# delehef/asgart

Hardware: AMD Instinct MI355X
Metric: Mbp/s probe+extend (direct+RC, k=20 g=100) (higher is better)
Workload: dtype u64 keys / u32 SA

## Files before the change

asgart_amd/csrc/call_front.hpp:

```cpp
#pragma once
#include "search_call.hpp"

namespace asgart {

__global__ void stall_kernel(unsigned long long ticks) {
    const unsigned long long t0 = wall_clock64();
    while (wall_clock64() - t0 < ticks) __builtin_amdgcn_s_sleep(100);
}

struct ProbeBuffer {
    DevBuf Workspace::*buf;
    size_t (*bytes)(uint64_t W, bool wide);
};
static const ProbeBuffer kProbeBuffers[7] = {
    {&Workspace::p_lo, [](uint64_t W, bool wide) { return (size_t)W * (wide ? 8 : 4); }},
    {&Workspace::p_raw, [](uint64_t W, bool) { return (size_t)W * 4; }},
    {&Workspace::p_filt, [](uint64_t W, bool) { return (size_t)W * 4; }},
    {&Workspace::row_off, [](uint64_t W, bool) { return ((size_t)W + 1) * 8; }},
    {&Workspace::blk, [](uint64_t W, bool) { return (size_t)((W + kScanTile - 1) / kScanTile + 4) * sizeof(ScanEl); }},
    {&Workspace::big_list, [](uint64_t W, bool) { return (size_t)W * 4; }},
    {&Workspace::rank_list, [](uint64_t W, bool) { return (size_t)W * 4; }},
};

int32_t reserve_probe_workspace(asgart_index *idx, SearchCtx &cx, uint64_t W) {
    Workspace &w = cx.ws;
    for (const ProbeBuffer &pb : kProbeBuffers)
        if (pb.buf != &Workspace::rank_list || idx->d_sap) RC_TRY((w.*pb.buf).reserve(pb.bytes(W, idx->wide)));
    RC_TRY(w.counters.reserve(CT_COUNT * 8));
    return 0;
}

bool carve_probe_workspace(asgart_index *idx, const uint64_t *Wc) {
    if (idx->ws_arena.p) return false;
    size_t off = 0;
    struct Piece {
        DevBuf *b;
// ... 26 lines not shown
    const uint32_t n_blk = rp.n_tiles((uint32_t)kScanTile);
    const uint64_t seg_cap = (uint64_t)W_probes / (rp.tstar + 1) + (uint64_t)n_chunks + 64;
    RC_TRY(reserve_probe_workspace(idx, cx, W));
    RC_TRY(w.seg_list.reserve((size_t)seg_cap * 4));
    RC_TRY(w.counters.reserve(CT_COUNT * 8));
    d_ctr = w.counters.as<unsigned long long>();
    HIP_TRY(hipMemsetAsync(d_ctr, 0, CT_COUNT * 8, s));
    ix = idx->template view<SlotT>();
    p_lo = w.p_lo.as<SlotT>() - rp.g_lo;
    p_raw = w.p_raw.as<uint32_t>() - rp.g_lo;
    p_filt = w.p_filt.as<uint32_t>() - rp.g_lo;
    row_off = w.row_off.as<unsigned long long>() - rp.g_lo;
    unsigned long long *scan_desc = w.blk.as<unsigned long long>();
    uint32_t *big_list = w.big_list.as<uint32_t>();
    uint32_t *rank_list = w.rank_list.as<uint32_t>();
    seg_list = w.seg_list.as<uint32_t>();

    if (opt.test_stall_s > 0) stall_kernel<<<1, 64, 0, s>>>((unsigned long long)opt.test_stall_s * 100000000ull);
    HIP_TRY(hipEventRecord(cx.ev[EV_SEARCH], s));
    probe_count_kernel<SlotT, false><<<rp.n_tiles((uint32_t)kProbeBlock), kProbeThreads, 0, s>>>(
        ix, rp, p_lo, p_raw, p_filt, big_list, rank_list, d_ctr);
    HIP_TRY(hipEventRecord(cx.ev[EV_PROBE_COUNT], s));
    collect_pending_kernel<<<std::min<uint32_t>(rp.n_tiles((uint32_t)kCollectTile), 256u * 8u), kCollectBlock, 0, s>>>(
        rp, p_filt, big_list, rank_list, d_ctr);
    big_count_kernel<SlotT, false><<<2048, 256, 0, s>>>(ix, rp, p_lo, p_raw, p_filt, big_list, d_ctr);
    uint32_t *const ranked_top = big_list + W;
    if (ix.sap)
        rank_count_kernel<SlotT, false><<<2048, 256, 0, s>>>(ix, rp, p_lo, p_raw, p_filt, rank_list, big_list, ranked_top,
                                                             ix.sar ? idx->ranked_fill : 0, d_ctr);
    HIP_TRY(hipEventRecord(cx.ev[EV_SEARCHED], s));
    HIP_TRY(hipMemsetAsync(scan_desc, 0, (size_t)n_blk * 16, s));
    scan_segments_kernel<<<std::min<uint32_t>(n_blk, 256u * 2u), kScanBlock, 0, s>>>(rp, p_filt, scan_desc, n_blk, row_off, seg_list, d_ctr);
    HIP_TRY(hipEventRecord(cx.ev[EV_SCANNED], s));
    HIP_TRY(hipGetLastError());
    HIP_TRY(hipMemcpyAsync(h_ctr, d_ctr, kCtrBytes, hipMemcpyDeviceToHost, s));
    RC_TRY(wd_sync(idx, cx, s, "the probe search and the scans"));
    total_hits = h_ctr[CT_TOTAL_HITS];
    n_seg = h_ctr[CT_SEG];
    if (h_ctr[CT_AMBIG]) {
// ... 49 lines not shown
```

asgart_amd/csrc/call_place.hpp:

```cpp
#pragma once
#include "search_call.hpp"

namespace asgart {

template <class SlotT>
int32_t SearchCall<SlotT>::place() {
    rec_cap = std::max<uint64_t>(1u << 18, w.fam_sds.cap / sizeof(SdRec));
    RC_TRY(w.ovf_list.reserve((size_t)(n_seg + 1) * 4 * kTiers));
    h_recs = nullptr;
    n_hrec = 0;
    const int force_tier = (int)opt.force_tier;
    RC_TRY(w.seg_keys.reserve((size_t)n_seg * 4 * 2));
    RC_TRY(w.seg_vals.reserve((size_t)n_seg * 4 * 2));
    uint32_t *kbuf = w.seg_keys.as<uint32_t>(), *vbuf = w.seg_vals.as<uint32_t>();
    HIP_TRY(hipMemsetAsync(d_ctr + CT_N1, 0, (size_t)(CT_COUNT - CT_N1) * 8, s));
    arms_kernel = rp.C <= (uint64_t)kHitBatch && opt.arms_kernel != 0 && (uint64_t)idx->n < (1ull << 42);
    for (int t = 1; t <= kTiers; ++t) {
        const TierShape &sh = shape(t);
        const bool usable = sh.kernel != TierKernel::none && !(arms_kernel && rp.C > (uint64_t)sh.hits);
        tier_cap[t] = usable ? (uint32_t)((uint64_t)sh.cap() * (uint64_t)(sh.widen ? opt.*sh.widen : 100) / 100u) : 0u;
    }
    tier_cap[kTiers] = 0xFFFFFFFFu;
    if (arms_kernel)
        tier_cap[3] = std::min(std::max(shape(3).cap(), tier_cap[6]), tier_cap[3]);
// ... 46 lines not shown
    int force_eff = force_tier;
    while (force_eff > 1 && force_eff < kTiers && !tier_enabled(force_eff)) ++force_eff;
    pp.sum1 = kTier1MaxSum;
    pp.force_tier = force_eff;
    {
        uint32_t *long_list = w.ovf_list.as<uint32_t>();
        seg_stats_lanes_kernel<<<(unsigned)std::min<uint64_t>((n_seg + 63) / 64, 256ull * 9ull * 2ull), 64, 0, s>>>(
            rp, p_filt, seg_list, d_ctr + CT_SEG, kbuf, vbuf, pp, long_list, d_ctr);
        seg_stats_kernel<<<(unsigned)std::min<uint64_t>(n_seg, 256ull * 16ull), 64, 0, s>>>(
            rp, p_filt, seg_list, d_ctr + CT_LONGSEG, long_list, kbuf, vbuf, pp, d_ctr);
    }
    HIP_TRY(hipGetLastError());
    HIP_TRY(hipStreamWaitEvent(s, cx.ev[EV_HIT_ROWS], 0));
    if (cluster_barren) {
        HIP_TRY(hipEventRecord(cx.ev[EV_BARREN], s));
        cluster_barren_kernel<SlotT, 16384><<<256 * 32, 64, 0, s>>>(rp, pp, row_off, hits, seg_list, d_ctr + CT_SEG, kbuf, 1u, 1024u,
                                                                   d_ctr + CT_CLUSTER_CUR, d_ctr);
        HIP_TRY(hipEventRecord(cx.ev[EV_BARREN_SMALL], s));
        cluster_barren_kernel<SlotT, 131072><<<256 * 9, 64, 0, s>>>(rp, pp, row_off, hits, seg_list, d_ctr + CT_SEG, kbuf, 1025u,
                                                                   16384u, d_ctr + CT_CLUSTER_CUR + 1, d_ctr);
        HIP_TRY(hipGetLastError());
        HIP_TRY(hipEventRecord(cx.ev[EV_BARREN_BIG], s));
    }
    if (split_on) {
        SplitParams sp{};
        sp.range_len = (uint32_t)opt.split_len;
        sp.warm = (uint32_t)opt.split_warm;
        sp.min_span = (uint32_t)std::min<int64_t>(opt.split_min, 0x7FFFFFFF);
        sp.max_runs = kMaxRuns - kMaxSplits;
        sp.max_cuts = kMaxCuts;
        sp.max_splits = kMaxSplits;
        {
            BlockedSeg *h_blocked = reinterpret_cast<BlockedSeg *>(h_split + kOffBlocked);
            std::lock_guard<std::mutex> lk(idx->mu);
            sp.n_blocked = blocked_in_call(idx->split_blocked, call_sig, rp.modes, n_passes, lo_lim, hi_lim, kSplitBlockedMax,
                                           [&](int32_t p_, const SplitVerdict &b) {
                                               *h_blocked++ = BlockedSeg{(uint32_t)p_ * K + ((uint32_t)b.key - lo_lim), b.range_len, b.allowed, b.warm};
// ... 80 lines not shown
        fprintf(stderr, "[asgart] %u long segment(s) cut into ranges: %u runs (ranges of %llu probes%s), %u cuts to check\n",
                n_splits, n_runs, (unsigned long long)h_split_hdr[4], opt.split_len ? "" : ": the shortest that keeps the runs within the budget", n_cuts);
    if (opt.debug) {
        fprintf(stderr, "[asgart] %llu segments, %llu walked wave by wave; per tier:", (unsigned long long)n_seg,
                (unsigned long long)h_ctr[CT_LONGSEG]);
        unsigned long long placed = 0;
        for (int t = 0; t < kTiers; ++t) {
            fprintf(stderr, " %llu", (unsigned long long)n_t[t]);
            placed += n_t[t];
        }
        fprintf(stderr, "; %llu barren (no arm can reach min_duplication_length: not run), %llu of them by the positions of their hits\n",
                (unsigned long long)n_seg - placed, (unsigned long long)h_ctr[CT_CLUSTER_BARREN]);
        fprintf(stderr, "[asgart] tail rule: thresholds (hits) of tiers 2, 4, 5: %u %u %u; %llu segment(s) moved to the next tier that holds more\n",
                pp.tail_hits[1], pp.tail_hits[3], pp.tail_hits[4], (unsigned long long)h_ctr[CT_TAIL_UP]);
        if (cluster_barren) {
            float ms_a = 0.f, ms_b = 0.f, ms_p = 0.f;
            (void)hipEventElapsedTime(&ms_a, cx.ev[EV_BARREN], cx.ev[EV_BARREN_SMALL]);
            (void)hipEventElapsedTime(&ms_b, cx.ev[EV_BARREN_SMALL], cx.ev[EV_BARREN_BIG]);
            (void)hipEventElapsedTime(&ms_p, cx.ev[EV_FILL], cx.ev[EV_BARREN]);
            fprintf(stderr, "[asgart] hit rows filled, placement walk beside it: %.2f ms; barren by position: segments of up to 1 024 hits %.2f ms, up to 16 384 hits %.2f ms\n",
                    ms_p, ms_a, ms_b);
        }
    }
    for (int t = 0; t < kTiers; ++t) ovf[t] = w.ovf_list.as<uint32_t>() + (size_t)t * (n_seg + 1);
    heavy_cap64 = (std::max<uint64_t>((uint64_t)rp.C * ((uint64_t)rp.tstar + 1u) + 64u, 4096u) + 3u) & ~3ull;
    if (heavy_cap64 >= (1ull << 24)) {
        set_error("max_cardinality * (max_gap_size / step + 1) = %llu live arms per segment: more than 2^24 are not supported",
                  (unsigned long long)heavy_cap64);
        return ASGART_E_CAP;
    }
    const size_t per_wg7 = (size_t)heavy_cap64 * (4 * sizeof(SlotT) + 28);
    const size_t per_wg6 = (size_t)caph * (4 * sizeof(SlotT) + 16);
    const size_t per_wg = std::max(per_wg6, per_wg7);
    n_wg7 = (unsigned)std::max<uint64_t>(1, std::min<uint64_t>(256, (16ull << 30) / (4 * per_wg)));
    region = std::max(per_wg6 * 256, per_wg * (size_t)n_wg7);
    RC_TRY(w.scratch.reserve(region * 4));
// ... 7 lines not shown
```

asgart_amd/csrc/call_stats.hpp:

```cpp
#pragma once
#include "search_call.hpp"

using namespace asgart;

template <class F>
static void by_slot(const asgart_index *idx, F f) {
    if (idx->wide) f(uint64_t{});
    else f(uint32_t{});
}

extern "C" {

int32_t asgart_tier_segments(asgart_index *idx, uint64_t *out) {
    if (!idx || !out) {
        set_error("bad argument");
        return ASGART_E_ARG;
    }
    idx->acquire_all();
    const SearchCtx &cx = idx->ctx[idx->last_ctx];
    for (int i = 0; i < 8; ++i) out[i] = cx.has_last ? cx.tier_segments[i] : 0;
    idx->release_all();
    return 0;
}

// ... 115 lines not shown
            }
            const unsigned g = rp.n_tiles(256u);
            by_slot(idx, [&](auto slot_tag) {
                using SlotT = decltype(slot_tag);
                yardstick_kernel<SlotT><<<g, 256, 0, s>>>(idx->view<SlotT>(), rp, cx.ws.p_filt.as<uint32_t>() - rp.g_lo, d_ctr);
            });
            HIP_TRY(hipGetLastError());
            HIP_TRY(hipMemsetAsync(d_ctr + CT_ALG_BYTES, 0, 16, s));
            HIP_TRY(hipMemsetAsync(d_ctr + CT_ALG_BYTES16, 0, 8, s));
            HIP_TRY(hipMemsetAsync(d_ctr + CT_LOOKUP_ACCT, 0, (size_t)LA_COUNT * 8, s));
            const unsigned gp = rp.n_tiles((uint32_t)kProbeBlock);
            by_slot(idx, [&](auto slot_tag) {
                using SlotT = decltype(slot_tag);
                IndexView<SlotT> ix = idx->view<SlotT>();
                probe_count_kernel<SlotT, true><<<gp, kProbeThreads, 0, s>>>(
                    ix, rp, nullptr, nullptr, nullptr, nullptr, nullptr, d_ctr);
                big_count_kernel<SlotT, true><<<2048, 256, 0, s>>>(
                    ix, rp, cx.ws.p_lo.as<SlotT>() - rp.g_lo, cx.ws.p_raw.as<uint32_t>() - rp.g_lo, nullptr,
                    cx.ws.big_list.as<uint32_t>(), d_ctr);
                if (ix.sap)
                    rank_count_kernel<SlotT, true><<<2048, 256, 0, s>>>(
                        ix, rp, cx.ws.p_lo.as<SlotT>() - rp.g_lo, cx.ws.p_raw.as<uint32_t>() - rp.g_lo, nullptr,
                        cx.ws.rank_list.as<uint32_t>(), nullptr, nullptr, 0, d_ctr);
            });
            HIP_TRY(hipGetLastError());
            unsigned long long v = 0, ab[2] = {0, 0}, a16 = 0;
            HIP_TRY(read_back(&v, d_ctr + CT_BISECT, 8, s));
            HIP_TRY(read_back(ab, d_ctr + CT_ALG_BYTES, 16, s));
            HIP_TRY(read_back(&a16, d_ctr + CT_ALG_BYTES16, 8, s));
            unsigned long long la[LA_COUNT];
            HIP_TRY(read_back(la, d_ctr + CT_LOOKUP_ACCT, sizeof(la), s));
// ... 17 lines not shown
```

asgart_amd/csrc/index.hpp:

```cpp
#pragma once

#include "common.hpp"
#include "range_join.hpp"
#include "run_dir.hpp"

#include <functional>
#include <memory>
#include <thread>
#include <condition_variable>
#include <mutex>

namespace asgart {

template <class SlotT>
struct IndexView {
    const uint8_t *text;
    const SlotT *sa;
    const uint64_t *keys;
    const SlotT *ptab;
    const SlotT *c8lo;
    const SlotT *c8hi;
    uint64_t n;
    int k;
    int kk;
// ... 79 lines not shown
    uint32_t create_seq;
    uint32_t pad;
    asgart_proto_sd sd;
};

struct Workspace {
    DevBuf chunks;
    DevBuf p_lo;
    DevBuf p_raw;
    DevBuf p_filt;
    DevBuf row_off;
    DevBuf blk;
    DevBuf hits;
    DevBuf big_list;
    DevBuf rank_list;
    DevBuf seg_list;
    DevBuf counters;
    DevBuf fam_sds;
    DevBuf ovf_list;
    DevBuf scratch;
    DevBuf seg_keys, seg_vals, sort_tmp;
    DevBuf rec_k32, rec_k64, rec_idx, rec_sorted;
    DevBuf pat;
    DevBuf out_a, out_b;
    DevBuf seg_info;
    DevBuf seg_slots;
    DevBuf split_buf;
    DevBuf split_dump;
    void release_all() {
        DevBuf *bufs[] = {&chunks, &p_lo, &p_raw, &p_filt, &row_off, &blk, &hits, &big_list, &rank_list, &seg_list,
                          &counters, &fam_sds, &ovf_list, &scratch, &seg_keys, &seg_vals,
                          &sort_tmp, &rec_k32, &rec_k64, &rec_idx, &rec_sorted, &pat, &out_a, &out_b, &seg_info, &seg_slots, &split_buf, &split_dump};
        static_assert(sizeof(Workspace) == sizeof(bufs) / sizeof(bufs[0]) * sizeof(DevBuf),
                      "a buffer of the workspace is missing from release_all");
        for (DevBuf *b : bufs) b->release();
    }
};

}

namespace asgart {
enum CtxEvent {
    EV_SEARCH,
    EV_PROBE_COUNT,
    EV_SEARCHED,
    EV_SCANNED,
    EV_FILL,
    EV_HIT_ROWS,
    EV_BARREN,
    EV_BARREN_SMALL,
    EV_BARREN_BIG,
    EV_TIERS,
    EV_EXTENDED,
    EV_COUNT
};
struct SearchCtx {
    static constexpr int kMaxTierStreams = 6;
    hipStream_t stream = nullptr;
    hipStream_t tier_st[kMaxTierStreams] = {};
    int n_tier_st = 0;
    hipStream_t fill_stream = nullptr;
    hipEvent_t ev[EV_COUNT] = {};
    hipEvent_t tier_ev[7] = {};
    hipEvent_t runs_ev = nullptr;
    uint64_t plan_sig = 0;
    bool plan_known = false;
// ... 390 lines not shown
```

asgart_amd/csrc/place_dev.hpp:

```cpp
#pragma once

#include "device_base.hpp"

namespace asgart {

struct PlaceParams {
    uint32_t cap[kTiers - 1];
    uint32_t sum1;
    int force_tier;
    uint32_t long3;
    uint32_t long3_big;
    uint32_t dense6;
    uint32_t stats;
    uint32_t barren;
    uint2 *seg_info;
    uint32_t k, step, G;
    unsigned long long M;
    uint32_t dense3;
    uint32_t tail_hits[kTiers - 1];
};

constexpr int kTierBarren = kTiers + 1;
__device__ inline bool segment_is_barren(const PlaceParams &pp, uint32_t n_hit, uint32_t span_probes) {
    if (!pp.barren || n_hit == 0u) return false;
// ... 212 lines not shown
            if (tail_up && tier != kTierBarren) atomicAdd(&ctr[CT_TAIL_UP], 1ull);
            keys[sidx] = placement_key(tier, sum, g0);
            vals[sidx] = g0;
            if (pp.seg_info)
                pp.seg_info[sidx] = make_uint2(sum > 0xFFFFFFFFull ? 0xFFFFFFFFu : (uint32_t)sum,
                                               (min(g_stop, g_end) - g0) | ((done || !window_cut) ? 0x80000000u : 0u));
            if (pp.stats) {
                atomicAdd(&ctr[CT_TPROBES1 + tier - 1], (unsigned long long)n_hit);
                atomicAdd(&ctr[CT_THITS1 + tier - 1], sum);
            }
        }
        lds_barrier();
    }
}

template <class PosT, int BITS>
__global__ __launch_bounds__(64) void cluster_barren_kernel(RunParams rp, PlaceParams pp,
                                                            const unsigned long long *__restrict__ row_off,
                                                            const PosT *__restrict__ hits,
                                                            const uint32_t *__restrict__ seg_list,
                                                            const unsigned long long *__restrict__ n_seg_ptr,
                                                            uint32_t *__restrict__ keys, uint32_t min_hits, uint32_t max_hits,
                                                            unsigned long long *__restrict__ cursor,
                                                            unsigned long long *__restrict__ ctr) {
    static_assert((BITS & (BITS - 1)) == 0 && BITS >= 2048, "bitmap size");
    constexpr uint32_t kWords = BITS / 32, kShift = 32 - __builtin_ctz((unsigned)BITS);
    __shared__ uint32_t s_bits[kWords];
    const uint32_t lane = threadIdx.x;
    const uint64_t n_seg = *n_seg_ptr;
    uint32_t n_barren = 0;
    auto bit_of = [&](uint32_t b) { return (b * 2654435761u) >> kShift; };
    for (;;) {
        unsigned long long base = 0;
        if (lane == 0) base = atomicAdd(cursor, 64ull);
        base = lane_of(base, 0u);
        if (base >= n_seg) break;
        const uint64_t sj = base + lane;
        bool cand = false;
        uint32_t key_l = 0, span_l = 0;
        unsigned long long lo_l = 0, hi_l = 0;
        if (sj < n_seg) {
            key_l = keys[sj];
            const uint2 info = pp.seg_info[sj];
            span_l = info.y & 0x7FFFFFFFu;
            cand = (key_l >> 29) < (uint32_t)kTiers && (info.y >> 31) && info.x >= min_hits && info.x <= max_hits;
            if (cand) {
                const uint32_t g0 = seg_list[sj];
                lo_l = row_off[g0];
                hi_l = row_off[g0 + span_l];
                cand = hi_l > lo_l && hi_l - lo_l <= (unsigned long long)max_hits;
            }
        }
        unsigned long long todo = __ballot(cand);
        while (todo) {
            const uint32_t l = (uint32_t)(__ffsll((long long)todo) - 1);
            todo &= todo - 1ull;
            const uint32_t key = lane_of(key_l, l), span = lane_of(span_l, l);
            const unsigned long long lo = lane_of(lo_l, l);
            const uint32_t n = (uint32_t)(lane_of(hi_l, l) - lo);
            const unsigned long long len_left_max = (unsigned long long)span * pp.step + pp.k;
            const unsigned long long thr_max = max((unsigned long long)pp.G, len_left_max / 10ull);
            const unsigned long long w = thr_max + pp.k;
            const unsigned long long need = (pp.M - pp.k) / w + 1ull;
            if (need < 2ull || need > 64ull) continue;
            const double inv_w = 1.0 / (double)w;
            auto bucket_of = [&](unsigned long long x) -> uint32_t {
                unsigned long long q = (unsigned long long)((double)x * inv_w);
                const long long r = (long long)(x - q * w);
                q += r >= (long long)w ? 1ull : 0ull;
                q -= r < 0 ? 1ull : 0ull;
                return (uint32_t)q;
            };
            for (uint32_t j = lane; j < kWords; j += 64u) s_bits[j] = 0u;
            __builtin_amdgcn_wave_barrier();
            __asm__ volatile("s_waitcnt lgkmcnt(0)" ::: "memory");
            for (uint32_t j0 = 0; j0 < n; j0 += 512u) {
                PosT xv[8];
#pragma unroll
                for (int u = 0; u < 8; ++u) {
                    const uint32_t j = j0 + (uint32_t)u * 64u + lane;
                    xv[u] = j < n ? hits[lo + j] : (PosT)0;
                }
#pragma unroll
                for (int u = 0; u < 8; ++u) {
                    const uint32_t j = j0 + (uint32_t)u * 64u + lane;
                    if (j < n) {
                        const uint32_t bi = bit_of(bucket_of((unsigned long long)xv[u]));
                        atomicOr(&s_bits[bi >> 5], 1u << (bi & 31u));
                    }
                }
            }
            __asm__ volatile("s_waitcnt lgkmcnt(0)" ::: "memory");
            __builtin_amdgcn_wave_barrier();
            bool found = false;
            for (uint32_t j0 = 0; j0 < n && !found; j0 += 512u) {
                PosT xv[8];
#pragma unroll
                for (int u = 0; u < 8; ++u) {
                    const uint32_t j = j0 + (uint32_t)u * 64u + lane;
                    xv[u] = j < n ? hits[lo + j] : (PosT)0;
                }
                bool mine = false;
#pragma unroll
                for (int u = 0; u < 8; ++u) {
                    const uint32_t j = j0 + (uint32_t)u * 64u + lane;
                    if (j < n) {
                        const uint32_t b = bucket_of((unsigned long long)xv[u]);
                        bool all = true;
                        for (uint32_t d = 1; d < (uint32_t)need && all; ++d) {
                            const uint32_t bi = bit_of(b + d);
                            all = (s_bits[bi >> 5] >> (bi & 31u)) & 1u;
                        }
                        mine = mine || all;
                    }
                }
                found = __ballot(mine) != 0ull;
            }
            __builtin_amdgcn_wave_barrier();
            if (!found) {
                if (lane == 0) keys[base + l] = (key & 0x1FFFFFFFu) | ((uint32_t)(kTierBarren - 1) << 29);
                ++n_barren;
            }
        }
    }
    if (lane == 0 && n_barren) atomicAdd(&ctr[CT_CLUSTER_BARREN], (unsigned long long)n_barren);
}

__global__ void tier_bounds_kernel(const uint32_t *__restrict__ sorted_keys,
                                   const unsigned long long *__restrict__ n_seg_ptr,
                                   unsigned long long *__restrict__ ctr) {
    const int t = threadIdx.x;
    if (t >= kTiers) return;
    const uint64_t n = *n_seg_ptr;
    auto first_ge = [&](uint32_t tier_idx) {
        uint64_t lo = 0, hi = n;
        while (lo < hi) {
// ... 10 lines not shown
```

asgart_amd/csrc/probe_dev.hpp:

```cpp
#pragma once

#include "device_base.hpp"

namespace asgart {

constexpr int kProbeBlock = 256;
constexpr int kProbeThreads = 64;
constexpr int kProbeSub = kProbeBlock / kProbeThreads;
constexpr int kMaxHalf = (kMaxKey + 1) / 2;
constexpr int kWinBytes = ((kProbeBlock + 2) * kMaxHalf + 15 + 16 + 15) / 16 * 16;

template <class SlotT, bool COUNT>
__global__ __launch_bounds__(kProbeThreads) void probe_count_kernel(IndexView<SlotT> ix, RunParams rp,
                                                                    SlotT *__restrict__ p_lo,
                                                                    uint32_t *__restrict__ p_raw,
                                                                    uint32_t *__restrict__ p_filt,
                                                                    uint32_t *__restrict__ big_list,
                                                                    uint32_t *__restrict__ rank_list,
                                                                    unsigned long long *__restrict__ ctr) {
    __shared__ __attribute__((aligned(16))) uint8_t s_text[kWinBytes];
    __shared__ uint32_t s_half[kProbeBlock + 2];
    constexpr int kPbLoads = (kProbeBlock * kMaxHalf + 127) / 128 + 2;
    __shared__ __attribute__((aligned(16))) uint32_t s_pb[kPbLoads * 4];
    __shared__ uint8_t s_surv[kProbeBlock];
    typename std::conditional<COUNT, CountBytes, NoBytes>::type cb;
    const uint32_t lane = threadIdx.x;
    const unsigned long long lt_mask = (1ull << lane) - 1ull;
    uint32_t g_end;
    const uint32_t gb = rp.tile_of(blockIdx.x, (uint32_t)kProbeBlock, g_end);
    const uint32_t g_last = min(gb + (uint32_t)kProbeBlock, g_end) - 1u;
    const int k = rp.k, H = rp.step;
    const int c0 = chunk_of_uniform(rp.ch, gb);
    const bool uniform = rp.ch.pbase[c0 + 1] > g_last && k <= kMaxKey;
    uint32_t n_rej = 0;
    auto lookup = [&](uint32_t g_, uint64_t q_, uint64_t q2_, const ProbeAt &at_, const uint64_t *lrn_) {
        const bool reverse = (at_.md & 2u) != 0u, complement = (at_.md & 1u) != 0u;
        const HitRule hr = hit_rule(at_);
        uint64_t lo, hi;
        ProbeRef pr;
        pr.p = reverse ? ix.text + at_.s + at_.L - 1u - at_.i : ix.text + at_.s + at_.i;
        pr.dir = reverse ? -1 : 1;
        pr.comp = complement;
        const bool all_occurrences = kmer_range(ix, q_, q2_, pr, lo, hi, cb);
        const uint64_t raw = hi - lo;
        cb.looked_up(raw);
        if (!COUNT) {
            p_lo[g_] = (SlotT)lo;
            p_raw[g_] = (uint32_t)raw;
        }
// ... 7 lines not shown
                const uint64_t x = ix.sa[r];
                cnt += hr.keeps(x) ? 1u : 0u;
                if (reverse) any |= x >= hr.thr;
            }
            if (!reverse) any = cnt != 0u;
            if (!COUNT) p_filt[g_] = cnt > rp.C ? kSkipCard : cnt;
            cb.wr(4);
            if constexpr (!COUNT) {
                if (lrn_ && all_occurrences && !any) {
                    const uint64_t p = (uint64_t)probe_bit_pos(at_, k);
                    atomicAnd(const_cast<unsigned long long *>(reinterpret_cast<const unsigned long long *>(lrn_)) + (p >> 6),
                              ~(1ull << (p & 63u)));
                }
            }
        } else {
            if (!COUNT) p_filt[g_] = (ix.sap && all_occurrences && raw > (uint64_t)kRankMin) ? kPendingRank : kPending;
            cb.wr(4 + 4);
            cb.rd(4);
        }
    };
    auto screen = [&](uint32_t g_, uint32_t first_, bool pass_, uint32_t md_) {
        if (first_ == 4u) {
            if (!COUNT) p_filt[g_] = kSkipN;
            cb.wr(4);
            return false;
        }
        if (!pass_) {
            if (!COUNT) {
                p_raw[g_] = kRawUnknown;
                p_filt[g_] = 0u;
            }
            cb.wr(8);
            n_rej += 1;
// ... 70 lines not shown
                    const uint32_t b = (uint32_t)(probe_bit_pos(at_of(t), k) - pb_lo);
                    pass = (s_pb[b >> 5] >> (b & 31u)) & 1u;
                }
                survivor = screen(g, first, pass, md);
            }
            const unsigned long long sm = __ballot(survivor);
            if (survivor) s_surv[n_surv + (uint32_t)__popcll(sm & lt_mask)] = (uint8_t)t;
            n_surv += (uint32_t)__popcll(sm);
        }
        __syncthreads();
        for (uint32_t j = lane; j < n_surv; j += kProbeThreads) {
            const uint32_t t = s_surv[j];
            lookup(gb + t, key_of(t), 0ull, at_of(t), pbits);
        }
    } else {
#pragma unroll 1
        for (int u = 0; u < kProbeSub; ++u) {
            const uint32_t g = gb + lane + (uint32_t)u * kProbeThreads;
            if (g >= g_end) continue;
            const int c = chunk_of(rp.ch, g);
            const ProbeAt at = probe_at(rp, c, g);
            const uint64_t *const pbits = rp.pbits[rp.pass_of(c)];
            uint32_t first = 0;
            uint64_t q2 = 0;
            const uint64_t q = probe_key(ix.text, at.s, at.L, at.i, k, (at.md & 2u) != 0u, (at.md & 1u) != 0u, &first, &q2);
            cb.rd((uint32_t)k);
            bool pass = true;
            if (first != 4u && pbits) {
                const uint64_t p = (uint64_t)probe_bit_pos(at, k);
                cb.rd(8);
                pass = (pbits[p >> 6] >> (p & 63u)) & 1ull;
            }
            if (screen(g, first, pass, at.md)) lookup(g, q, q2, at, pbits);
        }
    }
    if constexpr (COUNT) {
        unsigned long long b = cb.n, r = n_rej, b16 = cb.n16;
        for (int off = 32; off > 0; off >>= 1) {
            b += __shfl_down(b, off);
            r += __shfl_down(r, off);
            b16 += __shfl_down(b16, off);
        }
        if (lane == 0) {
            atomicAdd(&ctr[CT_ALG_BYTES], b);
            if (r) atomicAdd(&ctr[CT_FLT_REJECTED], r);
            if (b16) atomicAdd(&ctr[CT_ALG_BYTES16], b16);
        }
        for (int j = 0; j < (int)LA_COUNT; ++j) {
            unsigned long long a = cb.la[j];
            for (int off = 32; off > 0; off >>= 1) a += __shfl_down(a, off);
            if (lane == 0 && a) atomicAdd(&ctr[CT_LOOKUP_ACCT + j], a);
        }
    }
}

constexpr int kCollectBlock = 256, kCollectItems = 8, kCollectTile = kCollectBlock * kCollectItems;
constexpr int kCollectCap = 2 * kCollectTile;
__global__ __launch_bounds__(kCollectBlock) void collect_pending_kernel(RunParams rp, const uint32_t *__restrict__ p_filt,
                                                                        uint32_t *__restrict__ big_list,
                                                                        uint32_t *__restrict__ rank_list,
                                                                        unsigned long long *__restrict__ ctr) {
    __shared__ uint32_t s_buf[2][kCollectCap];
    __shared__ uint32_t s_cnt[2];
    __shared__ unsigned long long s_base[2];
    const uint32_t tid = threadIdx.x, lane = tid & 63u;
    const unsigned long long lt_mask = (1ull << lane) - 1ull;
    if (tid < 2) s_cnt[tid] = 0;
    __syncthreads();
    const uint32_t n_tiles = rp.n_tiles((uint32_t)kCollectTile);
    const uint32_t t0 = (uint32_t)((uint64_t)n_tiles * blockIdx.x / gridDim.x);
    const uint32_t t1 = (uint32_t)((uint64_t)n_tiles * (blockIdx.x + 1u) / gridDim.x);
    auto flush = [&](int which, uint32_t *__restrict__ list, int counter) {
        const uint32_t n = s_cnt[which];
        if (!n) return;
        if (tid == 0) s_base[which] = atomicAdd(&ctr[counter], (unsigned long long)n);
        __syncthreads();
        const unsigned long long b = s_base[which];
        for (uint32_t j = tid; j < n; j += kCollectBlock) list[b + j] = s_buf[which][j];
        __syncthreads();
        if (tid == 0) s_cnt[which] = 0;
        __syncthreads();
    };
    for (uint32_t t = t0; t < t1; ++t) {
        uint32_t g_end;
        const uint32_t g0 = rp.tile_of(t, (uint32_t)kCollectTile, g_end);
#pragma unroll
        for (int a = 0; a < kCollectItems; ++a) {
            const uint32_t g = g0 + (uint32_t)a * kCollectBlock + tid;
            const uint32_t f = g < g_end ? p_filt[g] : 0u;
            const bool big = f == kPending, rank = f == kPendingRank;
            const unsigned long long mb = __ballot(big), mr = __ballot(rank);
            if (mb) {
                uint32_t base = 0;
                if (lane == 0) base = atomicAdd(&s_cnt[0], (uint32_t)__popcll(mb));
                base = (uint32_t)__builtin_amdgcn_readfirstlane((int)base);
                if (big) s_buf[0][base + (uint32_t)__popcll(mb & lt_mask)] = g;
            }
            if (mr) {
                uint32_t base = 0;
                if (lane == 0) base = atomicAdd(&s_cnt[1], (uint32_t)__popcll(mr));
                base = (uint32_t)__builtin_amdgcn_readfirstlane((int)base);
                if (rank) s_buf[1][base + (uint32_t)__popcll(mr & lt_mask)] = g;
            }
        }
        __syncthreads();
        const uint32_t c0 = s_cnt[0], c1 = s_cnt[1];
        __syncthreads();
        if (c0 > (uint32_t)(kCollectCap - kCollectTile)) flush(0, big_list, CT_BIG);
        if (c1 > (uint32_t)(kCollectCap - kCollectTile)) flush(1, rank_list, CT_RANK);
    }
    flush(0, big_list, CT_BIG);
    flush(1, rank_list, CT_RANK);
}

template <class SlotT, bool COUNT>
__global__ __launch_bounds__(256) void rank_count_kernel(IndexView<SlotT> ix, RunParams rp,
                                                         const SlotT *__restrict__ p_lo,
// ... 199 lines not shown
```

Baseline: 53870.

## Collect pending probes from per-block bitmasks and merge barren clustering launches

The probe kernel now records pending (big/rank) probe positions in a per-block shared bitmask and writes it to a compact pend_mask buffer. The collect kernel reads these masks instead of rescanning the whole p_filt array, using a wave prefix sum to compact positions. Separately, the two barren-clustering launches (small and big segments) are merged into one 256-thread kernel where each wave owns a quarter of a shared bitmap and big segments are handled cooperatively. This adds an extra workspace buffer and an extra block-wide barrier in the probe kernel.

New measurement: 55190, median of 6. 1.02x the previous value.

```diff
diff --git a/asgart_amd/csrc/call_front.hpp b/asgart_amd/csrc/call_front.hpp
--- a/asgart_amd/csrc/call_front.hpp
+++ b/asgart_amd/csrc/call_front.hpp
@@ -12,7 +12,7 @@
     DevBuf Workspace::*buf;
     size_t (*bytes)(uint64_t W, bool wide);
 };
-static const ProbeBuffer kProbeBuffers[7] = {
+static const ProbeBuffer kProbeBuffers[8] = {
     {&Workspace::p_lo, [](uint64_t W, bool wide) { return (size_t)W * (wide ? 8 : 4); }},
     {&Workspace::p_raw, [](uint64_t W, bool) { return (size_t)W * 4; }},
     {&Workspace::p_filt, [](uint64_t W, bool) { return (size_t)W * 4; }},
@@ -20,6 +20,7 @@
     {&Workspace::blk, [](uint64_t W, bool) { return (size_t)((W + kScanTile - 1) / kScanTile + 4) * sizeof(ScanEl); }},
     {&Workspace::big_list, [](uint64_t W, bool) { return (size_t)W * 4; }},
     {&Workspace::rank_list, [](uint64_t W, bool) { return (size_t)W * 4; }},
+    {&Workspace::pend_mask, [](uint64_t W, bool) { return (size_t)(W / kProbeBlock + 8) * kPendMaskBytes; }},
 };
 
 int32_t reserve_probe_workspace(asgart_index *idx, SearchCtx &cx, uint64_t W) {
@@ -76,15 +77,16 @@
     unsigned long long *scan_desc = w.blk.as<unsigned long long>();
     uint32_t *big_list = w.big_list.as<uint32_t>();
     uint32_t *rank_list = w.rank_list.as<uint32_t>();
+    uint32_t *pend_mask = w.pend_mask.as<uint32_t>();
     seg_list = w.seg_list.as<uint32_t>();
 
     if (opt.test_stall_s > 0) stall_kernel<<<1, 64, 0, s>>>((unsigned long long)opt.test_stall_s * 100000000ull);
     HIP_TRY(hipEventRecord(cx.ev[EV_SEARCH], s));
     probe_count_kernel<SlotT, false><<<rp.n_tiles((uint32_t)kProbeBlock), kProbeThreads, 0, s>>>(
-        ix, rp, p_lo, p_raw, p_filt, big_list, rank_list, d_ctr);
+        ix, rp, p_lo, p_raw, p_filt, pend_mask, d_ctr);
     HIP_TRY(hipEventRecord(cx.ev[EV_PROBE_COUNT], s));
-    collect_pending_kernel<<<std::min<uint32_t>(rp.n_tiles((uint32_t)kCollectTile), 256u * 8u), kCollectBlock, 0, s>>>(
-        rp, p_filt, big_list, rank_list, d_ctr);
+    collect_pending_kernel<<<std::min<uint32_t>(collect_units(rp), 256u * 8u), kCollectBlock, 0, s>>>(
+        rp, pend_mask, big_list, rank_list, d_ctr);
     big_count_kernel<SlotT, false><<<2048, 256, 0, s>>>(ix, rp, p_lo, p_raw, p_filt, big_list, d_ctr);
     uint32_t *const ranked_top = big_list + W;
     if (ix.sap)
diff --git a/asgart_amd/csrc/call_place.hpp b/asgart_amd/csrc/call_place.hpp
--- a/asgart_amd/csrc/call_place.hpp
+++ b/asgart_amd/csrc/call_place.hpp
@@ -84,13 +84,10 @@
     HIP_TRY(hipStreamWaitEvent(s, cx.ev[EV_HIT_ROWS], 0));
     if (cluster_barren) {
         HIP_TRY(hipEventRecord(cx.ev[EV_BARREN], s));
-        cluster_barren_kernel<SlotT, 16384><<<256 * 32, 64, 0, s>>>(rp, pp, row_off, hits, seg_list, d_ctr + CT_SEG, kbuf, 1u, 1024u,
-                                                                   d_ctr + CT_CLUSTER_CUR, d_ctr);
-        HIP_TRY(hipEventRecord(cx.ev[EV_BARREN_SMALL], s));
-        cluster_barren_kernel<SlotT, 131072><<<256 * 9, 64, 0, s>>>(rp, pp, row_off, hits, seg_list, d_ctr + CT_SEG, kbuf, 1025u,
-                                                                   16384u, d_ctr + CT_CLUSTER_CUR + 1, d_ctr);
+        cluster_barren_kernel<SlotT><<<(unsigned)std::clamp<uint64_t>((n_seg + kBarrenBatch - 1) / kBarrenBatch, 1ull, 256ull * 8ull), kBarrenBlock, 0, s>>>(
+            rp, pp, row_off, hits, seg_list, d_ctr + CT_SEG, kbuf, d_ctr + CT_CLUSTER_CUR, d_ctr);
         HIP_TRY(hipGetLastError());
-        HIP_TRY(hipEventRecord(cx.ev[EV_BARREN_BIG], s));
+        HIP_TRY(hipEventRecord(cx.ev[EV_BARREN_DONE], s));
     }
     if (split_on) {
         SplitParams sp{};
@@ -201,12 +198,11 @@
         fprintf(stderr, "[asgart] tail rule: thresholds (hits) of tiers 2, 4, 5: %u %u %u; %llu segment(s) moved to the next tier that holds more\n",
                 pp.tail_hits[1], pp.tail_hits[3], pp.tail_hits[4], (unsigned long long)h_ctr[CT_TAIL_UP]);
         if (cluster_barren) {
-            float ms_a = 0.f, ms_b = 0.f, ms_p = 0.f;
-            (void)hipEventElapsedTime(&ms_a, cx.ev[EV_BARREN], cx.ev[EV_BARREN_SMALL]);
-            (void)hipEventElapsedTime(&ms_b, cx.ev[EV_BARREN_SMALL], cx.ev[EV_BARREN_BIG]);
+            float ms_b = 0.f, ms_p = 0.f;
+            (void)hipEventElapsedTime(&ms_b, cx.ev[EV_BARREN], cx.ev[EV_BARREN_DONE]);
             (void)hipEventElapsedTime(&ms_p, cx.ev[EV_FILL], cx.ev[EV_BARREN]);
-            fprintf(stderr, "[asgart] hit rows filled, placement walk beside it: %.2f ms; barren by position: segments of up to 1 024 hits %.2f ms, up to 16 384 hits %.2f ms\n",
-                    ms_p, ms_a, ms_b);
+            fprintf(stderr, "[asgart] hit rows filled, placement walk beside it: %.2f ms; barren by position (segments of up to 16 384 hits, one launch): %.2f ms\n",
+                    ms_p, ms_b);
         }
     }
     for (int t = 0; t < kTiers; ++t) ovf[t] = w.ovf_list.as<uint32_t>() + (size_t)t * (n_seg + 1);
diff --git a/asgart_amd/csrc/call_stats.hpp b/asgart_amd/csrc/call_stats.hpp
--- a/asgart_amd/csrc/call_stats.hpp
+++ b/asgart_amd/csrc/call_stats.hpp
@@ -153,7 +153,7 @@
                 using SlotT = decltype(slot_tag);
                 IndexView<SlotT> ix = idx->view<SlotT>();
                 probe_count_kernel<SlotT, true><<<gp, kProbeThreads, 0, s>>>(
-                    ix, rp, nullptr, nullptr, nullptr, nullptr, nullptr, d_ctr);
+                    ix, rp, nullptr, nullptr, nullptr, nullptr, d_ctr);
                 big_count_kernel<SlotT, true><<<2048, 256, 0, s>>>(
                     ix, rp, cx.ws.p_lo.as<SlotT>() - rp.g_lo, cx.ws.p_raw.as<uint32_t>() - rp.g_lo, nullptr,
                     cx.ws.big_list.as<uint32_t>(), d_ctr);
diff --git a/asgart_amd/csrc/index.hpp b/asgart_amd/csrc/index.hpp
--- a/asgart_amd/csrc/index.hpp
+++ b/asgart_amd/csrc/index.hpp
@@ -117,6 +117,7 @@
     DevBuf hits;
     DevBuf big_list;
     DevBuf rank_list;
+    DevBuf pend_mask;
     DevBuf seg_list;
     DevBuf counters;
     DevBuf fam_sds;
@@ -131,7 +132,7 @@
     DevBuf split_buf;
     DevBuf split_dump;
     void release_all() {
-        DevBuf *bufs[] = {&chunks, &p_lo, &p_raw, &p_filt, &row_off, &blk, &hits, &big_list, &rank_list, &seg_list,
+        DevBuf *bufs[] = {&chunks, &p_lo, &p_raw, &p_filt, &row_off, &blk, &hits, &big_list, &rank_list, &pend_mask, &seg_list,
                           &counters, &fam_sds, &ovf_list, &scratch, &seg_keys, &seg_vals,
                           &sort_tmp, &rec_k32, &rec_k64, &rec_idx, &rec_sorted, &pat, &out_a, &out_b, &seg_info, &seg_slots, &split_buf, &split_dump};
         static_assert(sizeof(Workspace) == sizeof(bufs) / sizeof(bufs[0]) * sizeof(DevBuf),
@@ -151,8 +152,7 @@
     EV_FILL,
     EV_HIT_ROWS,
     EV_BARREN,
-    EV_BARREN_SMALL,
-    EV_BARREN_BIG,
+    EV_BARREN_DONE,
     EV_TIERS,
     EV_EXTENDED,
     EV_COUNT
diff --git a/asgart_amd/csrc/place_dev.hpp b/asgart_amd/csrc/place_dev.hpp
--- a/asgart_amd/csrc/place_dev.hpp
+++ b/asgart_amd/csrc/place_dev.hpp
@@ -250,112 +250,221 @@
     }
 }
 
-template <class PosT, int BITS>
-__global__ __launch_bounds__(64) void cluster_barren_kernel(RunParams rp, PlaceParams pp,
-                                                            const unsigned long long *__restrict__ row_off,
-                                                            const PosT *__restrict__ hits,
-                                                            const uint32_t *__restrict__ seg_list,
-                                                            const unsigned long long *__restrict__ n_seg_ptr,
-                                                            uint32_t *__restrict__ keys, uint32_t min_hits, uint32_t max_hits,
-                                                            unsigned long long *__restrict__ cursor,
-                                                            unsigned long long *__restrict__ ctr) {
-    static_assert((BITS & (BITS - 1)) == 0 && BITS >= 2048, "bitmap size");
-    constexpr uint32_t kWords = BITS / 32, kShift = 32 - __builtin_ctz((unsigned)BITS);
+constexpr uint32_t kBarrenSmallHits = 1024, kBarrenBigHits = 16384;
+constexpr int kBarrenBlock = 256, kBarrenWaves = kBarrenBlock / 64, kBarrenBatch = kBarrenWaves * 64;
+constexpr int kBarrenSmallBits = 16384, kBarrenBigBits = 131072, kBarrenList = 16;
+struct BarrenBig {
+    unsigned long long lo;
+    uint32_t n, key, span, at;
+};
+template <class PosT>
+__global__ __launch_bounds__(kBarrenBlock, sizeof(PosT) == 4 ? 8 : 4) void cluster_barren_kernel(RunParams rp, PlaceParams pp,
+                                                                      const unsigned long long *__restrict__ row_off,
+                                                                      const PosT *__restrict__ hits,
+                                                                      const uint32_t *__restrict__ seg_list,
+                                                                      const unsigned long long *__restrict__ n_seg_ptr,
+                                                                      uint32_t *__restrict__ keys,
+                                                                      unsigned long long *__restrict__ cursor,
+                                                                      unsigned long long *__restrict__ ctr) {
+    constexpr uint32_t kWords = kBarrenBigBits / 32, kQuarter = kWords / kBarrenWaves, kSmallWords = kBarrenSmallBits / 32;
+    constexpr uint32_t kSmallShift = 32 - __builtin_ctz((unsigned)kBarrenSmallBits), kBigShift = 32 - __builtin_ctz((unsigned)kBarrenBigBits);
+    static_assert(kSmallWords <= kQuarter, "a wave's bitmap lies inside its quarter");
     __shared__ uint32_t s_bits[kWords];
-    const uint32_t lane = threadIdx.x;
+    __shared__ BarrenBig s_list[kBarrenList];
+    __shared__ unsigned long long s_base;
+    __shared__ uint32_t s_nlist, s_found;
+    const uint32_t tid = threadIdx.x, lane = tid & 63u, wave = tid >> 6;
+    uint32_t *const my_bits = s_bits + wave * kQuarter;
     const uint64_t n_seg = *n_seg_ptr;
     uint32_t n_barren = 0;
-    auto bit_of = [&](uint32_t b) { return (b * 2654435761u) >> kShift; };
+    if (tid == 0) s_found = 0u;
+    auto need_of = [&](uint32_t span, unsigned long long &w) {
+        const unsigned long long len_left_max = (unsigned long long)span * pp.step + pp.k;
+        const unsigned long long thr_max = max((unsigned long long)pp.G, len_left_max / 10ull);
+        w = thr_max + pp.k;
+        return (pp.M - pp.k) / w + 1ull;
+    };
+    auto bucket_of = [](unsigned long long x, unsigned long long w, double inv_w) -> uint32_t {
+        unsigned long long q = (unsigned long long)((double)x * inv_w);
+        const long long r = (long long)(x - q * w);
+        q += r >= (long long)w ? 1ull : 0ull;
+        q -= r < 0 ? 1ull : 0ull;
+        return (uint32_t)q;
+    };
+    const uint32_t barren_key = (uint32_t)(kTierBarren - 1) << 29;
     for (;;) {
-        unsigned long long base = 0;
-        if (lane == 0) base = atomicAdd(cursor, 64ull);
-        base = lane_of(base, 0u);
+        if (tid == 0) s_base = atomicAdd(cursor, (unsigned long long)kBarrenBatch);
+        __syncthreads();
+        const unsigned long long base = s_base;
         if (base >= n_seg) break;
-        const uint64_t sj = base + lane;
-        bool cand = false;
+        const uint64_t sj = base + tid;
+        bool cand = false, big = false;
         uint32_t key_l = 0, span_l = 0;
         unsigned long long lo_l = 0, hi_l = 0;
         if (sj < n_seg) {
             key_l = keys[sj];
             const uint2 info = pp.seg_info[sj];
             span_l = info.y & 0x7FFFFFFFu;
-            cand = (key_l >> 29) < (uint32_t)kTiers && (info.y >> 31) && info.x >= min_hits && info.x <= max_hits;
+            big = info.x > kBarrenSmallHits;
+            cand = (key_l >> 29) < (uint32_t)kTiers && (info.y >> 31) && info.x >= 1u && info.x <= kBarrenBigHits;
             if (cand) {
                 const uint32_t g0 = seg_list[sj];
                 lo_l = row_off[g0];
                 hi_l = row_off[g0 + span_l];
-                cand = hi_l > lo_l && hi_l - lo_l <= (unsigned long long)max_hits;
-            }
-        }
-        unsigned long long todo = __ballot(cand);
+                unsigned long long w;
+                const unsigned long long need = need_of(span_l, w);
+                cand = hi_l > lo_l && hi_l - lo_l <= (unsigned long long)(big ? kBarrenBigHits : kBarrenSmallHits) &&
+                       need >= 2ull && need <= 64ull;
+            }
+        }
+        unsigned long long todo = __ballot(cand && !big);
         while (todo) {
             const uint32_t l = (uint32_t)(__ffsll((long long)todo) - 1);
             todo &= todo - 1ull;
-            const uint32_t key = lane_of(key_l, l), span = lane_of(span_l, l);
+            const uint32_t key = lane_of(key_l, l);
             const unsigned long long lo = lane_of(lo_l, l);
             const uint32_t n = (uint32_t)(lane_of(hi_l, l) - lo);
-            const unsigned long long len_left_max = (unsigned long long)span * pp.step + pp.k;
-            const unsigned long long thr_max = max((unsigned long long)pp.G, len_left_max / 10ull);
-            const unsigned long long w = thr_max + pp.k;
-            const unsigned long long need = (pp.M - pp.k) / w + 1ull;
-            if (need < 2ull || need > 64ull) continue;
+            unsigned long long w;
+            const uint32_t need = (uint32_t)need_of(lane_of(span_l, l), w);
             const double inv_w = 1.0 / (double)w;
-            auto bucket_of = [&](unsigned long long x) -> uint32_t {
-                unsigned long long q = (unsigned long long)((double)x * inv_w);
-                const long long r = (long long)(x - q * w);
-                q += r >= (long long)w ? 1ull : 0ull;
-                q -= r < 0 ? 1ull : 0ull;
-                return (uint32_t)q;
-            };
-            for (uint32_t j = lane; j < kWords; j += 64u) s_bits[j] = 0u;
+            auto bit_of = [&](uint32_t b) { return (b * 2654435761u) >> kSmallShift; };
+            for (uint32_t j = lane; j < kSmallWords; j += 64u) my_bits[j] = 0u;
             __builtin_amdgcn_wave_barrier();
             __asm__ volatile("s_waitcnt lgkmcnt(0)" ::: "memory");
-            for (uint32_t j0 = 0; j0 < n; j0 += 512u) {
-                PosT xv[8];
+            PosT xa[8];
+            auto load8 = [&](PosT *xv, uint32_t j0) {
 #pragma unroll
                 for (int u = 0; u < 8; ++u) {
                     const uint32_t j = j0 + (uint32_t)u * 64u + lane;
                     xv[u] = j < n ? hits[lo + j] : (PosT)0;
                 }
+            };
+            auto set8 = [&](const PosT *xv, uint32_t j0) {
 #pragma unroll
                 for (int u = 0; u < 8; ++u) {
                     const uint32_t j = j0 + (uint32_t)u * 64u + lane;
                     if (j < n) {
-                        const uint32_t bi = bit_of(bucket_of((unsigned long long)xv[u]));
-                        atomicOr(&s_bits[bi >> 5], 1u << (bi & 31u));
-                    }
-                }
-            }
-            __asm__ volatile("s_waitcnt lgkmcnt(0)" ::: "memory");
-            __builtin_amdgcn_wave_barrier();
-            bool found = false;
-            for (uint32_t j0 = 0; j0 < n && !found; j0 += 512u) {
-                PosT xv[8];
-#pragma unroll
-                for (int u = 0; u < 8; ++u) {
-                    const uint32_t j = j0 + (uint32_t)u * 64u + lane;
-                    xv[u] = j < n ? hits[lo + j] : (PosT)0;
-                }
+                        const uint32_t bi = bit_of(bucket_of((unsigned long long)xv[u], w, inv_w));
+                        atomicOr(&my_bits[bi >> 5], 1u << (bi & 31u));
+                    }
+                }
+            };
+            auto test8 = [&](const PosT *xv, uint32_t j0) {
                 bool mine = false;
 #pragma unroll
                 for (int u = 0; u < 8; ++u) {
                     const uint32_t j = j0 + (uint32_t)u * 64u + lane;
                     if (j < n) {
-                        const uint32_t b = bucket_of((unsigned long long)xv[u]);
+                        const uint32_t b = bucket_of((unsigned long long)xv[u], w, inv_w);
                         bool all = true;
-                        for (uint32_t d = 1; d < (uint32_t)need && all; ++d) {
+                        for (uint32_t d = 1; d < need && all; ++d) {
                             const uint32_t bi = bit_of(b + d);
-                            all = (s_bits[bi >> 5] >> (bi & 31u)) & 1u;
+                            all = (my_bits[bi >> 5] >> (bi & 31u)) & 1u;
                         }
                         mine = mine || all;
                     }
                 }
-                found = __ballot(mine) != 0ull;
+                return __ballot(mine) != 0ull;
+            };
+            load8(xa, 0u);
+            set8(xa, 0u);
+            if (n > 512u) {
+                PosT xb[8];
+                load8(xb, 512u);
+                set8(xb, 512u);
+            }
+            __asm__ volatile("s_waitcnt lgkmcnt(0)" ::: "memory");
+            __builtin_amdgcn_wave_barrier();
+            bool found = test8(xa, 0u);
+            if (!found && n > 512u) {
+                PosT xb[8];
+                load8(xb, 512u);
+                found = test8(xb, 512u);
             }
             __builtin_amdgcn_wave_barrier();
             if (!found) {
-                if (lane == 0) keys[base + l] = (key & 0x1FFFFFFFu) | ((uint32_t)(kTierBarren - 1) << 29);
+                if (lane == 0) keys[base + wave * 64u + l] = (key & 0x1FFFFFFFu) | barren_key;
                 ++n_barren;
+            }
+        }
+        unsigned long long big_todo = __ballot(cand && big);
+        for (;;) {
+            __syncthreads();
+            if (tid == 0) s_nlist = 0u;
+            __syncthreads();
+            while (big_todo) {
+                const uint32_t l = (uint32_t)(__ffsll((long long)big_todo) - 1);
+                uint32_t slot = 0;
+                if (lane == 0) slot = atomicAdd(&s_nlist, 1u);
+                slot = (uint32_t)__builtin_amdgcn_readfirstlane((int)slot);
+                if (slot >= (uint32_t)kBarrenList) break;
+                big_todo &= big_todo - 1ull;
+                if (lane == l) s_list[slot] = BarrenBig{lo_l, (uint32_t)(hi_l - lo_l), key_l, span_l, tid};
+            }
+            __syncthreads();
+            const uint32_t n_list = min(s_nlist, (uint32_t)kBarrenList);
+            if (!n_list) break;
+            for (uint32_t e = 0; e < n_list; ++e) {
+                const unsigned long long lo = s_list[e].lo;
+                const uint32_t n = s_list[e].n;
+                unsigned long long w;
+                const uint32_t need = (uint32_t)need_of(s_list[e].span, w);
+                const double inv_w = 1.0 / (double)w;
+                auto bit_of = [&](uint32_t b) { return (b * 2654435761u) >> kBigShift; };
+                for (uint32_t j = tid; j < kWords; j += (uint32_t)kBarrenBlock) s_bits[j] = 0u;
+                __syncthreads();
+                constexpr uint32_t kRound = 8u * (uint32_t)kBarrenBlock;
+                PosT xv[8];
+                for (uint32_t j0 = 0; j0 < n; j0 += kRound) {
+#pragma unroll
+                    for (int u = 0; u < 8; ++u) {
+                        const uint32_t j = j0 + (uint32_t)u * kBarrenBlock + tid;
+                        xv[u] = j < n ? hits[lo + j] : (PosT)0;
+                    }
+#pragma unroll
+                    for (int u = 0; u < 8; ++u) {
+                        const uint32_t j = j0 + (uint32_t)u * kBarrenBlock + tid;
+                        if (j < n) {
+                            const uint32_t bi = bit_of(bucket_of((unsigned long long)xv[u], w, inv_w));
+                            atomicOr(&s_bits[bi >> 5], 1u << (bi & 31u));
+                        }
+                    }
+                }
+                __syncthreads();
+                bool found = false;
+                for (uint32_t j0 = 0; j0 < n && !found; j0 += kRound) {
+                    if (n > kRound) {
+#pragma unroll
+                        for (int u = 0; u < 8; ++u) {
+                            const uint32_t j = j0 + (uint32_t)u * kBarrenBlock + tid;
+                            xv[u] = j < n ? hits[lo + j] : (PosT)0;
+                        }
+                    }
+                    bool mine = false;
+#pragma unroll
+                    for (int u = 0; u < 8; ++u) {
+                        const uint32_t j = j0 + (uint32_t)u * kBarrenBlock + tid;
+                        if (j < n) {
+                            const uint32_t b = bucket_of((unsigned long long)xv[u], w, inv_w);
+                            bool all = true;
+                            for (uint32_t d = 1; d < need && all; ++d) {
+                                const uint32_t bi = bit_of(b + d);
+                                all = (s_bits[bi >> 5] >> (bi & 31u)) & 1u;
+                            }
+                            mine = mine || all;
+                        }
+                    }
+                    found = __ballot(mine) != 0ull;
+                }
+                if (found && lane == 0) s_found = 1u;
+                __syncthreads();
+                if (tid == 0) {
+                    if (!s_found) {
+                        keys[base + s_list[e].at] = (s_list[e].key & 0x1FFFFFFFu) | barren_key;
+                        ++n_barren;
+                    }
+                    s_found = 0u;
+                }
             }
         }
     }
diff --git a/asgart_amd/csrc/probe_dev.hpp b/asgart_amd/csrc/probe_dev.hpp
--- a/asgart_amd/csrc/probe_dev.hpp
+++ b/asgart_amd/csrc/probe_dev.hpp
@@ -7,6 +7,7 @@
 constexpr int kProbeBlock = 256;
 constexpr int kProbeThreads = 64;
 constexpr int kProbeSub = kProbeBlock / kProbeThreads;
+constexpr int kPendMaskWords = 2 * kProbeBlock / 32, kPendMaskBytes = kPendMaskWords * 4;
 constexpr int kMaxHalf = (kMaxKey + 1) / 2;
 constexpr int kWinBytes = ((kProbeBlock + 2) * kMaxHalf + 15 + 16 + 15) / 16 * 16;
 
@@ -15,10 +16,10 @@
                                                                     SlotT *__restrict__ p_lo,
                                                                     uint32_t *__restrict__ p_raw,
                                                                     uint32_t *__restrict__ p_filt,
-                                                                    uint32_t *__restrict__ big_list,
-                                                                    uint32_t *__restrict__ rank_list,
+                                                                    uint32_t *__restrict__ pend_mask,
                                                                     unsigned long long *__restrict__ ctr) {
     __shared__ __attribute__((aligned(16))) uint8_t s_text[kWinBytes];
+    __shared__ uint32_t s_pend[kPendMaskWords];
     __shared__ uint32_t s_half[kProbeBlock + 2];
     constexpr int kPbLoads = (kProbeBlock * kMaxHalf + 127) / 128 + 2;
     __shared__ __attribute__((aligned(16))) uint32_t s_pb[kPbLoads * 4];
@@ -33,6 +34,7 @@
     const int c0 = chunk_of_uniform(rp.ch, gb);
     const bool uniform = rp.ch.pbase[c0 + 1] > g_last && k <= kMaxKey;
     uint32_t n_rej = 0;
+    if (lane < (uint32_t)kPendMaskWords) s_pend[lane] = 0u;
     auto lookup = [&](uint32_t g_, uint64_t q_, uint64_t q2_, const ProbeAt &at_, const uint64_t *lrn_) {
         const bool reverse = (at_.md & 2u) != 0u, complement = (at_.md & 1u) != 0u;
         const HitRule hr = hit_rule(at_);
@@ -70,9 +72,13 @@
                 }
             }
         } else {
-            if (!COUNT) p_filt[g_] = (ix.sap && all_occurrences && raw > (uint64_t)kRankMin) ? kPendingRank : kPending;
+            const bool by_rank = ix.sap && all_occurrences && raw > (uint64_t)kRankMin;
+            if (!COUNT) {
+                p_filt[g_] = by_rank ? kPendingRank : kPending;
+                const uint32_t t_ = g_ - gb;
+                atomicOr(&s_pend[(by_rank ? kPendMaskWords / 2 : 0) + (t_ >> 5)], 1u << (t_ & 31u));
+            }
             cb.wr(4 + 4);
-            cb.rd(4);
         }
     };
     auto screen = [&](uint32_t g_, uint32_t first_, bool pass_, uint32_t md_) {
@@ -173,6 +179,7 @@
             lookup(gb + t, key_of(t), 0ull, at_of(t), pbits);
         }
     } else {
+        __syncthreads();
 #pragma unroll 1
         for (int u = 0; u < kProbeSub; ++u) {
             const uint32_t g = gb + lane + (uint32_t)u * kProbeThreads;
@@ -193,6 +200,14 @@
             if (screen(g, first, pass, at.md)) lookup(g, q, q2, at, pbits);
         }
     }
+    if constexpr (!COUNT) {
+        __syncthreads();
+        if (lane < (uint32_t)kPendMaskWords) pend_mask[(size_t)blockIdx.x * kPendMaskWords + lane] = s_pend[lane];
+    }
+    if (lane == 0) {
+        cb.wr((uint32_t)kPendMaskBytes);
+        cb.rd((uint32_t)kPendMaskBytes);
+    }
     if constexpr (COUNT) {
         unsigned long long b = cb.n, r = n_rej, b16 = cb.n16;
         for (int off = 32; off > 0; off >>= 1) {
@@ -213,9 +228,13 @@
     }
 }
 
-constexpr int kCollectBlock = 256, kCollectItems = 8, kCollectTile = kCollectBlock * kCollectItems;
+constexpr int kCollectBlock = 256, kCollectTiles = 8, kCollectTile = kCollectTiles * kProbeBlock;
 constexpr int kCollectCap = 2 * kCollectTile;
-__global__ __launch_bounds__(kCollectBlock) void collect_pending_kernel(RunParams rp, const uint32_t *__restrict__ p_filt,
+static_assert(kCollectTiles * 2 * kProbeBlock == kCollectBlock * 16, "16 mask bits per thread and unit");
+__host__ __device__ inline uint32_t collect_units(const RunParams &rp) {
+    return (rp.n_tiles((uint32_t)kProbeBlock) + (uint32_t)kCollectTiles - 1u) / (uint32_t)kCollectTiles;
+}
+__global__ __launch_bounds__(kCollectBlock) void collect_pending_kernel(RunParams rp, const uint32_t *__restrict__ pend_mask,
                                                                         uint32_t *__restrict__ big_list,
                                                                         uint32_t *__restrict__ rank_list,
                                                                         unsigned long long *__restrict__ ctr) {
@@ -223,12 +242,11 @@
     __shared__ uint32_t s_cnt[2];
     __shared__ unsigned long long s_base[2];
     const uint32_t tid = threadIdx.x, lane = tid & 63u;
-    const unsigned long long lt_mask = (1ull << lane) - 1ull;
     if (tid < 2) s_cnt[tid] = 0;
     __syncthreads();
-    const uint32_t n_tiles = rp.n_tiles((uint32_t)kCollectTile);
-    const uint32_t t0 = (uint32_t)((uint64_t)n_tiles * blockIdx.x / gridDim.x);
-    const uint32_t t1 = (uint32_t)((uint64_t)n_tiles * (blockIdx.x + 1u) / gridDim.x);
+    const uint32_t n_ptiles = rp.n_tiles((uint32_t)kProbeBlock), n_units = collect_units(rp);
+    const uint32_t u0 = (uint32_t)((uint64_t)n_units * blockIdx.x / gridDim.x);
+    const uint32_t u1 = (uint32_t)((uint64_t)n_units * (blockIdx.x + 1u) / gridDim.x);
     auto flush = [&](int which, uint32_t *__restrict__ list, int counter) {
         const uint32_t n = s_cnt[which];
         if (!n) return;
@@ -240,26 +258,41 @@
         if (tid == 0) s_cnt[which] = 0;
         __syncthreads();
     };
-    for (uint32_t t = t0; t < t1; ++t) {
-        uint32_t g_end;
-        const uint32_t g0 = rp.tile_of(t, (uint32_t)kCollectTile, g_end);
-#pragma unroll
-        for (int a = 0; a < kCollectItems; ++a) {
-            const uint32_t g = g0 + (uint32_t)a * kCollectBlock + tid;
-            const uint32_t f = g < g_end ? p_filt[g] : 0u;
-            const bool big = f == kPending, rank = f == kPendingRank;
-            const unsigned long long mb = __ballot(big), mr = __ballot(rank);
-            if (mb) {
-                uint32_t base = 0;
-                if (lane == 0) base = atomicAdd(&s_cnt[0], (uint32_t)__popcll(mb));
-                base = (uint32_t)__builtin_amdgcn_readfirstlane((int)base);
-                if (big) s_buf[0][base + (uint32_t)__popcll(mb & lt_mask)] = g;
-            }
-            if (mr) {
-                uint32_t base = 0;
-                if (lane == 0) base = atomicAdd(&s_cnt[1], (uint32_t)__popcll(mr));
-                base = (uint32_t)__builtin_amdgcn_readfirstlane((int)base);
-                if (rank) s_buf[1][base + (uint32_t)__popcll(mr & lt_mask)] = g;
+    const uint16_t *const m16 = reinterpret_cast<const uint16_t *>(pend_mask);
+    const uint32_t sub = tid >> 5, which = (tid >> 4) & 1u, t_lo = (tid & 15u) * 16u;
+    auto load = [&](uint32_t u) -> uint32_t {
+        const uint32_t tile = u * (uint32_t)kCollectTiles + sub;
+        return u < u1 && tile < n_ptiles ? (uint32_t)m16[(size_t)tile * (kPendMaskWords * 2) + (tid & 31u)] : 0u;
+    };
+    uint32_t m_next = load(u0);
+    for (uint32_t u = u0; u < u1; ++u) {
+        uint32_t m = m_next;
+        m_next = load(u + 1u);
+        const uint32_t mine = (uint32_t)__popc(m) << (which ? 16u : 0u);
+        uint32_t incl = mine;
+#pragma unroll
+        for (int off = 1; off < 64; off <<= 1) {
+            const uint32_t v = __shfl_up(incl, off);
+            if ((int)lane >= off) incl += v;
+        }
+        const uint32_t tot = __shfl(incl, 63);
+        if (tot) {
+            uint32_t base_b = 0, base_r = 0;
+            if (lane == 0) {
+                if (tot & 0xFFFFu) base_b = atomicAdd(&s_cnt[0], tot & 0xFFFFu);
+                if (tot >> 16) base_r = atomicAdd(&s_cnt[1], tot >> 16);
+            }
+            base_b = (uint32_t)__builtin_amdgcn_readfirstlane((int)base_b);
+            base_r = (uint32_t)__builtin_amdgcn_readfirstlane((int)base_r);
+            if (m) {
+                uint32_t g_end;
+                const uint32_t g = rp.tile_of(u * (uint32_t)kCollectTiles + sub, (uint32_t)kProbeBlock, g_end) + t_lo;
+                const uint32_t before = incl - mine;
+                uint32_t at = which ? base_r + (before >> 16) : base_b + (before & 0xFFFFu);
+                while (m) {
+                    s_buf[which][at++] = g + (uint32_t)(__ffs((int)m) - 1);
+                    m &= m - 1u;
+                }
             }
         }
         __syncthreads();
```
